# DhayaaAnbajagane/Baryonification

Measured on AMD Instinct MI355X. Metric: halos/sec for BaryonifyShell NSIDE=1024 (1000000-halo synthetic catalog), higher is better.
Workload: dtype f64 throughout in the parity-grade mode: f64 ring-row geometry, f64 pair math with 1e-11 elementary functions (fp32 seeds + one Newton step), f64 LDS accumulation, pix_offsets stored as two f32 arrays (hi + lo), f64 regrid geometry, f64 map

## Files before the change

baryonification_amd/csrc/bfgx_kernels.hpp:

```cpp
#pragma once
#include <hip/hip_runtime.h>
#include <stdint.h>
#include "bfgx_cosmo.hpp"
#include "bfgx_math.hpp"

namespace bfgx {

constexpr double kTwoPi    = 6.283185307179586476925286766559005768394;
constexpr double kHalfPi   = 1.570796326794896619231321691639751442099;
constexpr double kInvTwoPi = 1.0 / kTwoPi;
constexpr double kTwoThird = 2.0 / 3.0;
constexpr double kDeg2Rad  = kPi / 180.0;
constexpr double kRad2Deg  = 180.0 / kPi;

constexpr int kWave = 64;
constexpr int kWavesPerBlock = 4;
constexpr int kNC = 4;

enum { MODE_OFFSETS = 0, MODE_PAINT = 1, MODE_COUNT = 2 };

struct Hpx {
    int64_t nside, npix, ncap;
    double fact1, fact2;
};
// ... 87 lines not shown
        const int64_t iphi = 4 * iring + 1 - (ip - 2 * iring * (iring - 1));
        const double tmp = (double)(iring * iring) * h.fact2;
        z = tmp - 1.0;
        sth = (z < -0.99) ? sqrt(tmp * (2.0 - tmp)) : sqrt((1.0 - z) * (1.0 + z));
        phi = ((double)iphi - 0.5) * kHalfPi / (double)iring;
    }
}

template <bool WANT_W>
__device__ inline void get_interpol_ring(const Hpx &h, int64_t ir1, double theta, double phi, int64_t pix[4], double wgt[4])
{
    const int64_t ir2 = ir1 + 1;
    double theta1 = 0.0, theta2 = 0.0;
    pix[0] = pix[1] = pix[2] = pix[3] = 0;
    wgt[0] = wgt[1] = wgt[2] = wgt[3] = 0.0;
#pragma unroll
    for (int half = 0; half < 2; ++half) {
        const int64_t ir = half ? ir2 : ir1;
        if (half ? (ir < 4 * h.nside) : (ir > 0)) {
            int64_t sp, nr; bool shifted; double th = 0.0;
            if (WANT_W) ring_info2(h, ir, sp, nr, th, shifted);
            else ring_info_small(h, ir, sp, nr, shifted);
            const double dphi = kTwoPi / (double)nr;
            const double sh = shifted ? 0.5 : 0.0;
            const double tmp = phi / dphi - sh;
            int64_t i1 = (tmp < 0) ? (int64_t)tmp - 1 : (int64_t)tmp;
            const double w1 = (phi - ((double)i1 + sh) * dphi) / dphi;
            int64_t i2 = i1 + 1;
            if (i1 < 0) i1 += nr;
            if (i2 >= nr) i2 -= nr;
            pix[2 * half] = sp + i1; pix[2 * half + 1] = sp + i2;
            wgt[2 * half] = 1.0 - w1; wgt[2 * half + 1] = w1;
            if (half) theta2 = th; else theta1 = th;
        }
    }
    if (ir1 == 0) {
        const double wtheta = theta / theta2;
        wgt[2] *= wtheta; wgt[3] *= wtheta;
        const double fac = (1.0 - wtheta) * 0.25;
        wgt[0] = fac; wgt[1] = fac; wgt[2] += fac; wgt[3] += fac;
        pix[0] = (pix[2] + 2) & 3;
        pix[1] = (pix[3] + 2) & 3;
    } else if (ir2 == 4 * h.nside) {
        const double wtheta = (theta - theta1) / (kPi - theta1);
        wgt[0] *= (1.0 - wtheta); wgt[1] *= (1.0 - wtheta);
        const double fac = wtheta * 0.25;
        wgt[0] += fac; wgt[1] += fac; wgt[2] = fac; wgt[3] = fac;
        pix[2] = ((pix[0] + 2) & 3) + h.npix - 4;
        pix[3] = ((pix[1] + 2) & 3) + h.npix - 4;
    } else {
        const double wtheta = (theta - theta1) / (theta2 - theta1);
        wgt[0] *= (1.0 - wtheta); wgt[1] *= (1.0 - wtheta);
        wgt[2] *= wtheta; wgt[3] *= wtheta;
    }
}

template <bool WANT_W>
__device__ inline void get_interpol(const Hpx &h, double theta, double phi, int64_t pix[4], double wgt[4])
{
    get_interpol_ring<WANT_W>(h, ring_above(h, cos(theta)), theta, phi, pix, wgt);
}


struct RowSpan {
    int64_t start, nr;
    int32_t lo, cnt;
    bool shifted;
    double z, sth;
};

__device__ inline void disc_row_span(int nr, bool shifted, double z, double fnr, int ring, double z0, double xa, double cosr,
                                     double phi0, int irmin, int irmax, int &lo, int &cnt)
{
    lo = 0; cnt = 0;
    if (ring < irmin || ring > irmax) { cnt = nr; return; }
    const double x = (cosr - z * z0) * xa;
    const double ysq = 1.0 - z * z - x * x;
    if (!(ysq > 0.0)) return;
    const double dphi = atan2(sqrt(ysq), x);
    if (!(dphi > 0.0)) return;
    const double sh = shifted ? 0.5 : 0.0;
    const int64_t ip_lo = (int64_t)floor(fnr * (phi0 - dphi) - sh) + 1;
    const int64_t ip_hi = (int64_t)floor(fnr * (phi0 + dphi) - sh);
    int64_t c = ip_hi - ip_lo + 1;
    c = c < 0 ? 0 : (c > nr ? nr : c);
    cnt = (int)c;
    int64_t l = ip_lo;
    if (l < 0) l += nr;
    if (l >= nr) l -= nr;
    if (l < 0) l += nr;
    lo = (int)l;
}

__device__ inline void disc_row(const Hpx &h, int ring, double z0, double xa, double cosr, double phi0,
                                int irmin, int irmax, RowSpan &s)
{
    ring_info_small(h, ring, s.start, s.nr, s.shifted);
    ring_z_sth(h, ring, s.z, s.sth);
    s.lo = 0; s.cnt = 0;
    if (ring < irmin || ring > irmax) { s.cnt = (int)s.nr; return; }
    const double x = (cosr - s.z * z0) * xa;
    const double ysq = 1.0 - s.z * s.z - x * x;
    if (!(ysq > 0.0)) return;
    const double dphi = atan2(sqrt(ysq), x);
    if (!(dphi > 0.0)) return;
    const double sh = s.shifted ? 0.5 : 0.0;
    const double fnr = (double)s.nr * kInvTwoPi;
    const int64_t ip_lo = (int64_t)floor(fnr * (phi0 - dphi) - sh) + 1;
    const int64_t ip_hi = (int64_t)floor(fnr * (phi0 + dphi) - sh);
    int64_t c = ip_hi - ip_lo + 1;
    c = c < 0 ? 0 : (c > s.nr ? s.nr : c);
    s.cnt = (int)c;
    int64_t l = ip_lo;
    if (l < 0) l += s.nr;
    if (l >= s.nr) l -= s.nr;
    if (l < 0) l += s.nr;
    s.lo = (int)l;
}

__device__ inline void interp_neighbours(const Hpx &h, double theta, double phi, int32_t ring[4], int32_t k[4])
{
    int64_t pix[4]; double w[4];
    get_interpol<false>(h, theta, phi, pix, w);
    const double z = cos(theta);
    const int64_t ir1 = ring_above(h, z), ir2 = ir1 + 1;
    for (int q = 0; q < 4; ++q) {
        int64_t rg = (q < 2) ? ir1 : ir2;
        if (rg < 1) rg = 1;
        if (rg > 4 * h.nside - 1) rg = 4 * h.nside - 1;
        int64_t st, nr; bool sh;
        ring_info_small(h, rg, st, nr, sh);
        ring[q] = (int32_t)rg;
        k[q] = (int32_t)(pix[q] - st);
    }
}

struct DevTable {
    int32_t ndim;
    int32_t n[BFGX_MAX_DIM];
    const double *axis[BFGX_MAX_DIM];
    const double *values;
    const float *values32;
    int32_t rdelta, logv;
    double eps_model;
    int32_t r_uniform;
    double r0, inv_dr, r1;
};

struct PairTable {
    const double *values, *raxis;
    const float *values32;
    double r0, inv_dr, r1;
    int32_t nr, r_uniform, rdelta, _pad;
};

__host__ __device__ inline PairTable make_pair_table(const DevTable &t)
{
    PairTable p;
    p.values = t.values; p.raxis = t.axis[2]; p.values32 = t.values32;
    p.r0 = t.r0; p.inv_dr = t.inv_dr; p.r1 = t.r1;
    p.nr = t.n[2]; p.r_uniform = t.r_uniform; p.rdelta = t.rdelta; p._pad = 0;
    return p;
}

struct DevModel {
    DevTable tab;
    Background bg_runner, bg_model;
    bfgx_massdef md_runner, md_model;
    double eps_runner;
    int32_t same_model;
    const double *da_coef;
    double da_step;
};

constexpr int kNCmax = 16;
constexpr int kNCmaxShell = 4 << BFGX_MAX_EXTRA;
struct RowSetX {
    double w[kNCmaxShell];
    int32_t rowoff[kNCmaxShell];
};
struct ExtraCols { const double *p[BFGX_MAX_EXTRA]; };

struct alignas(16) HaloRec {
    double z0, xa, s0, phi0;
    double cph0, sph0;
    double cosr;
    double theta, phi;
    double D, a, inv_a, rcut, lnoff;
    double w[kNC];
    int32_t rowoff[kNC];
    int32_t irmin, irmax, rfirst, rlast;
    int32_t oob;
    int32_t allphi;
    int32_t fb;
    int32_t _pad;
    double flo, fhi;
    int32_t fb_ring[4], fb_k[4];
};

__device__ inline double dev_E2(const Background &b, double a)
{
    const double a3 = a * a * a;
    const double de = (b.w0 == -1.0) ? b.Omega_l : b.Omega_l * pow(a, -3.0 * (1.0 + b.w0));
    return b.Omega_m / a3 + de + b.Omega_r / (a3 * a);
}

__device__ inline double dev_radius(const Background &b, const bfgx_massdef &md, double M, double a)
{
    double rho = b.rho_crit0 * dev_E2(b, a);
    if (md.rho_type == 1) rho = b.rho_crit0 * b.Omega_m / (a * a * a);
    return cbrt(M / (4.18879020479 * md.Delta * rho));
}

__device__ inline int axis_find(const double *g, int n, double x)
{
    if (!(x >= g[0]) || !(x <= g[n - 1])) return -1;
    int lo = 0, hi = n - 1;
    while (hi - lo > 1) {
        const int mid = (lo + hi) >> 1;
        if (x >= g[mid]) lo = mid; else hi = mid;
    }
    return lo;
}

template <int NC>
__device__ inline bool table_corners(const DevTable &tab, const double *gz, const double *gm, double x0, double x1, const double *xe,
                                     double *wv, int32_t *ro)
{
    const int iz = axis_find(gz, tab.n[0], x0);
    const int im = axis_find(gm, tab.n[1], x1);
    constexpr int K = (NC == 4) ? 0 : (NC == 8 ? 1 : (NC == 16 ? 2 : (NC == 32 ? 3 : 4)));
    static_assert(NC == (4 << K), "NC = 4 * 2^K");
    int ip[K > 0 ? K : 1];
    double tp[K > 0 ? K : 1];
    bool oob = (iz < 0 || im < 0);
#pragma unroll
    for (int k = 0; k < K; ++k) {
        const double *g = tab.axis[3 + k];
        ip[k] = axis_find(g, tab.n[3 + k], xe[k]);
        tp[k] = 0.0;
        oob = oob || ip[k] < 0;
        if (ip[k] >= 0) tp[k] = (xe[k] - g[ip[k]]) / (g[ip[k] + 1] - g[ip[k]]);
    }
    if (!oob) {
        const double tz = (x0 - gz[iz]) / (gz[iz + 1] - gz[iz]);
        const double tm = (x1 - gm[im]) / (gm[im + 1] - gm[im]);
        const int nr = tab.n[2];
        for (int c = 0; c < NC; ++c) {
            const int bz = (c >> (K + 1)) & 1, bm = (c >> K) & 1;
            double w = (1.0 * (bz ? tz : 1.0 - tz)) * (bm ? tm : 1.0 - tm);
            int idx = (iz + bz) * tab.n[1] + im + bm;
#pragma unroll
            for (int k = 0; k < K; ++k) {
                const int b = (c >> (K - 1 - k)) & 1;
                w *= (b ? tp[k] : 1.0 - tp[k]);
                idx = idx * tab.n[3 + k] + ip[k] + b;
            }
            wv[c] = w;
            ro[c] = idx * nr;
        }
    } else {
        for (int c = 0; c < NC; ++c) { wv[c] = 0.0; ro[c] = 0; }
    }
    return oob;
}

struct Tiling {
    int32_t BR, W, nbands, ntiles;
    const int32_t *band_tile0;
    const int32_t *band_nphi;
    const int32_t *band_nrmin;
    const int32_t *tile_band;
    const int32_t *tile_order;
    const struct RingRec *rings;
};

__device__ inline int tile_ks(int j, int nr, int nphi) { return (int)(((unsigned)j * (unsigned)nr + (unsigned)nphi - 1u) / (unsigned)nphi); }

__device__ inline int ring_len(const Hpx &h, int ring)
{
    const int64_t n = h.nside;
    return (int)(4 * (ring < n ? ring : (ring > 3 * n ? 4 * n - ring : n)));
}

constexpr int kRefMax = 4;
struct TileRef {
    union {
        struct { int32_t tile[kRefMax], slot[kRefMax]; } few;
        struct { int32_t rfirst, rlast, allphi, _p; double flo, fhi; } many;
    };
    int32_t n;
    int32_t live;
    int32_t _pad[2];
};

enum { kClsNone = 0, kClsFast = 1, kClsGeneric = 2 };

struct DiscSpan {
    int32_t fb, rfirst, rlast, allphi;
    int32_t fb_ring[4], fb_k[4];
    double flo, fhi;
};

template <typename F>
__device__ inline void for_each_tile(const Hpx &h, const Tiling &T, const DiscSpan &r, F &&f)
{
    if (r.fb) {
        int seen[4], ns = 0;
        for (int q = 0; q < 4; ++q) {
            const int b = (r.fb_ring[q] - 1) / T.BR;
            const int nphi = T.band_nphi[b];
            const int t = T.band_tile0[b] + (int)(((int64_t)r.fb_k[q] * nphi) / ring_len(h, r.fb_ring[q]));
            bool dup = false;
            for (int i = 0; i < ns; ++i) dup |= (seen[i] == t);
            if (!dup) { seen[ns++] = t; f(t); }
        }
        return;
    }
    if (r.rlast < r.rfirst) return;
    const int b0 = (r.rfirst - 1) / T.BR, b1 = (r.rlast - 1) / T.BR;
    for (int b = b0; b <= b1; ++b) {
        const int nphi = T.band_nphi[b], t0 = T.band_tile0[b];
        bool all = r.allphi || nphi == 1;
        int jlo = 0, jhi = nphi - 1;
        if (!all) {
            const double margin = 2.0 * (double)nphi / (double)T.band_nrmin[b] + 1e-6;
            jlo = (int)floor((double)nphi * r.flo - margin);
            jhi = (int)floor((double)nphi * r.fhi + margin);
            if (jhi - jlo + 1 >= nphi) { all = true; jlo = 0; jhi = nphi - 1; }
        }
        for (int jj = jlo; jj <= jhi; ++jj) {
            int j = jj % nphi;
            if (j < 0) j += nphi;
            f(t0 + j);
        }
    }
}

struct alignas(16) RowRec {
    double z0, s0, xa, cosr, phi0;
    int32_t rfirst, rlast;
    int32_t fb;
    int32_t _pad;
    double cut2;
};
struct FbRec { int32_t ring[4], k[4]; };

template <typename real>
struct alignas(16) PairRecT {
    real scale2;
    real cut2;
    real aD;
    real cph0, sph0;
    real w[4];
    int32_t cell;
    int32_t oob;
    int32_t hidx, _pad;
};

template <typename real>
struct Tab8T {
    const real *v;
    real r0, r1, inv_dr;
    int32_t nr, _pad;
};

constexpr int kCntPadMax = 32;
struct RunSlot { int base, hr; };
__device__ inline RunSlot wave_run_issue(int32_t *cnt, int tile, bool active)
{
    RunSlot r;
    r.base = 0; r.hr = 0;
    if (__ballot(active) == 0ull) return r;
    const int lane = (int)__builtin_amdgcn_mbcnt_hi(~0u, __builtin_amdgcn_mbcnt_lo(~0u, 0u));
    const int key = active ? tile : -1 - lane;
    const int prev = __shfl_up(key, 1, kWave);
    const bool head = (lane == 0) || (key != prev);
    const unsigned long long hm = __ballot(head);
    const int hl = 63 - __clzll((long long)(hm & ((2ull << lane) - 1ull)));
    const unsigned long long up = (lane == kWave - 1) ? 0ull : (hm >> (lane + 1));
    const int next = up ? lane + __ffsll((long long)up) : kWave;
    r.hr = active ? (hl | ((lane - hl + 1) << 8)) : 0;
    if (head && active) r.base = atomicAdd(cnt + tile, next - lane);
    return r;
}
__device__ inline int wave_run_resolve(const RunSlot &r)
{
    const int b = __shfl(r.base, r.hr & 63, kWave);
    return r.hr ? b + (r.hr >> 8) - 1 : 0;
}

struct PrepOut {
    HaloRec *rec;
    RowSetX *rowsx;
    RowRec *rowrec;
    void *pairrec;
    FbRec *fbrec;
    TileRef *tref;
    int32_t *cnt_a, *cnt_b;
    int32_t *entries_a, *slow_list, *slow_cnt;
    float *work_est;
    int32_t cap_a;
    int32_t cnt_pad;
    int32_t fast;
    int32_t rec_all;
    int32_t ncell_m, nrm1;
    int64_t blk_rows, blk_stride;
};

template <int NC, typename real>
__device__ __forceinline__ void halo_prep_one(const DevModel &m, const Hpx &h, int64_t j, bool live, const double *gz, const double *gm,
                                              const double *__restrict__ M, const double *__restrict__ z,
                                              const double *__restrict__ ra, const double *__restrict__ dec,
                                              ExtraCols ex,
                                              const double *__restrict__ lnz1, const double *__restrict__ lnM,
                                              int fallback4, const Tiling &T, const PrepOut &o, int *s_nslow, float *s_work);

constexpr int kK0Occ = 4;
template <int NC, typename real>
__global__ void __launch_bounds__(256, kK0Occ)
halo_prep_kernel(DevModel m, Hpx h, int64_t nhalo,
                 const double *__restrict__ M, const double *__restrict__ z,
                 const double *__restrict__ ra, const double *__restrict__ dec,
                 ExtraCols ex,
                 const double *__restrict__ lnz1, const double *__restrict__ lnM,
                 int fallback4, Tiling T, PrepOut o)
{
    __shared__ int s_nslow;
    __shared__ float s_work;
    if (threadIdx.x == 0) { s_nslow = 0; s_work = 0.0f; }
    constexpr int kAxisLds = 128;
    __shared__ double ax_lds[2 * kAxisLds];
    const bool ax_in_lds = m.tab.n[0] <= kAxisLds && m.tab.n[1] <= kAxisLds;
    if (ax_in_lds) {
        for (int i = threadIdx.x; i < m.tab.n[0]; i += blockDim.x) ax_lds[i] = m.tab.axis[0][i];
        for (int i = threadIdx.x; i < m.tab.n[1]; i += blockDim.x) ax_lds[kAxisLds + i] = m.tab.axis[1][i];
        __syncthreads();
    }
    const double *gz = ax_in_lds ? ax_lds : m.tab.axis[0], *gm = ax_in_lds ? ax_lds + kAxisLds : m.tab.axis[1];
    constexpr int kBandLds = 1024;
    __shared__ int32_t band_lds[3 * kBandLds + 1];
    if (o.tref && T.nbands <= kBandLds) {
        for (int i = threadIdx.x; i <= T.nbands; i += blockDim.x) band_lds[i] = T.band_tile0[i];
        for (int i = threadIdx.x; i < T.nbands; i += blockDim.x) { band_lds[kBandLds + 1 + i] = T.band_nphi[i]; band_lds[2 * kBandLds + 1 + i] = T.band_nrmin[i]; }
        __syncthreads();
        T.band_tile0 = band_lds; T.band_nphi = band_lds + kBandLds + 1; T.band_nrmin = band_lds + 2 * kBandLds + 1;
    }
    __syncthreads();
    const int64_t j = (int64_t)blockIdx.x * blockDim.x + threadIdx.x;
    halo_prep_one<NC, real>(m, h, j < nhalo ? j : nhalo - 1, j < nhalo, gz, gm, M, z, ra, dec, ex, lnz1, lnM, fallback4, T, o, &s_nslow, &s_work);
    if (o.slow_cnt) {
        __syncthreads();
        if (threadIdx.x == 0) o.slow_cnt[blockIdx.x] = s_nslow;
        if (threadIdx.x == 0 && o.work_est) o.work_est[blockIdx.x] = s_work;
    }
}

template <int NC, typename real>
__device__ __forceinline__ void halo_prep_one(const DevModel &m, const Hpx &h, int64_t j, bool live, const double *gz, const double *gm,
                                              const double *__restrict__ M, const double *__restrict__ z,
                                              const double *__restrict__ ra, const double *__restrict__ dec,
                                              ExtraCols ex,
                                              const double *__restrict__ lnz1, const double *__restrict__ lnM,
                                              int fallback4, const Tiling &T, const PrepOut &o, int *s_nslow, float *s_work)
{
    HaloRec r;
    const int64_t jin = o.blk_rows > 0 ? (j / o.blk_rows) * o.blk_stride + (j % o.blk_rows) : j;
    const double M_j = M[jin], z_j = z[jin];
    const double a = 1.0 / (1.0 + z_j);
    const double R = dev_radius(m.bg_runner, m.md_runner, M_j, a);
    double D;
    {
        int i = (int)floor(z_j / m.da_step);
        i = max(0, min(i, kDaKnots - 2));
        const double t = z_j - (double)i * m.da_step;
        const double *c = m.da_coef + 4 * i;
        D = ((c[0] * t + c[1]) * t + c[2]) * t + c[3];
    }
    const double radius = R * m.eps_runner / D;

    const double theta = kHalfPi - dec[jin] * kDeg2Rad;
    const double phi = ra[jin] * kDeg2Rad;
    double st, ct, sp, cp;
    sincos_bounded(theta, st, ct);
    sincos_bounded(phi, sp, cp);
    const double thq = theta;
    double phq = phi - kTwoPi * floor(phi * kInvTwoPi);
    if (phq >= kTwoPi) phq -= kTwoPi;
    if (st == 0.0) phq = 0.0;
    r.z0 = ct;
    r.s0 = st;
    r.xa = 1.0 / sqrt((1.0 - r.z0) * (1.0 + r.z0));
    r.phi0 = phq;
    r.cph0 = cp; r.sph0 = sp;
    r.theta = theta; r.phi = phi;
    r.D = D; r.a = a;

    const int64_t nl4 = 4 * h.nside;
    bool pole = false;
    double sr_ = 0.0;
    const bool bad = !live || !(radius > 0.0) || !isfinite(radius) || !(theta >= 0.0) || !(theta <= kPi) || !isfinite(phi);
    if (bad) {
        r.cosr = 1.0; r.irmin = 1; r.irmax = 0; r.rfirst = 1; r.rlast = 0;
        r.z0 = 1.0; r.s0 = 0.0; r.xa = 1.0; r.phi0 = 0.0; r.cph0 = 1.0; r.sph0 = 0.0;
    } else if (radius >= kPi) {
        r.cosr = -1.0; r.irmin = (int32_t)nl4; r.irmax = 0; r.rfirst = 1; r.rlast = (int32_t)(nl4 - 1);
        pole = true;
    } else {
        double cr_;
        sincos_bounded(radius, sr_, cr_);
        r.cosr = cr_;
        const double rlat1 = thq - radius;
        const double rlat2 = thq + radius;
        int64_t irmin = ring_above(h, ct * cr_ + st * sr_) + 1;
        int64_t irmax = ring_above(h, ct * cr_ - st * sr_);
        if (irmax > nl4 - 1) irmax = nl4 - 1;
        r.irmin = (int32_t)irmin; r.irmax = (int32_t)irmax;
        r.rfirst = (int32_t)(((rlat1 <= 0) && (irmin > 1)) ? 1 : irmin);
        r.rlast = (int32_t)(((rlat2 >= kPi) && (irmax + 1 < nl4)) ? nl4 - 1 : irmax);
        pole = (rlat1 <= 0) || (rlat2 >= kPi);
    }
    double dmax;
    {
        const double sr = (radius >= kHalfPi) ? 1.0 : sr_;
        r.allphi = (pole || radius >= kHalfPi || !(sr < 0.999 * r.s0)) ? 1 : 0;
        const double xs = sr / r.s0, xs2 = xs * xs;
        const double as_small = xs * (1.0 + xs2 * (1.0 / 6.0 + xs2 * (3.0 / 40.0 + xs2 * (15.0 / 336.0 + xs2 * (105.0 / 3456.0)))));
        dmax = r.allphi ? kPi : (xs < 0.35 ? as_small * (1.0 + 2e-6) : asin(xs));
        r.flo = (phq - dmax) * kInvTwoPi;
        r.fhi = (phq + dmax) * kInvTwoPi;
    }

    r.fb = 0; r._pad = 0;
    for (int q = 0; q < 4; ++q) { r.fb_ring[q] = 0; r.fb_k[q] = 0; }
    if (fallback4 && !bad && (r.rlast - r.rfirst) < 8) {
        int total = 0;
        const int span = r.rlast - r.rfirst, mid = (r.rfirst + r.rlast) >> 1;
        for (int t = 0; t <= span && total < 4; ++t) {
            const int ring = mid + ((t & 1) ? ((t + 1) >> 1) : -(t >> 1));
            RowSpan s;
            disc_row(h, ring, r.z0, r.xa, r.cosr, r.phi0, r.irmin, r.irmax, s);
            total += s.cnt;
        }
        if (total < 4) {
            r.fb = 1;
            interp_neighbours(h, theta, phi, r.fb_ring, r.fb_k);
        }
    }

    const bool to_fast = o.fast && NC == 4;
    const int cls = bad ? kClsNone : (to_fast ? kClsFast : kClsGeneric);
    bool geo_wide = false;
    if (cls == kClsFast) {
        geo_wide = r.allphi || !(dmax <= 0.40);
        if (r.fb) for (int q = 0; q < 4; ++q) if (r.fb_ring[q] < 16 || r.fb_ring[q] > (int)nl4 - 16) geo_wide = true;
    }
    if (o.work_est) {
        float w = (cls == kClsFast) ? (r.fb ? 4.0f : (float)(radius * radius) * 0.25f * (float)h.npix) : 0.0f;
#pragma unroll
        for (int sft = kWave >> 1; sft > 0; sft >>= 1) w += __shfl_xor(w, sft, kWave);
        if ((threadIdx.x & (kWave - 1)) == 0) atomicAdd(s_work, w);
    }
    TileRef ref;
    RunSlot run[kRefMax];
    for (int i = 0; i < kRefMax; ++i) { run[i].base = 0; run[i].hr = 0; }
    ref.n = 0; ref.live = cls != kClsNone; ref._pad[0] = ref._pad[1] = 0;
    for (int i = 0; i < kRefMax; ++i) { ref.few.tile[i] = 0; ref.few.slot[i] = 0; }
    if (o.tref) {
        DiscSpan ds;
        ds.fb = r.fb; ds.rfirst = r.rfirst; ds.rlast = r.rlast; ds.allphi = r.allphi; ds.flo = r.flo; ds.fhi = r.fhi;
        for (int q = 0; q < 4; ++q) { ds.fb_ring[q] = r.fb_ring[q]; ds.fb_k[q] = r.fb_k[q]; }
        int tl[kRefMax] = {0, 0, 0, 0};
        int nt = 0;
        if (cls != kClsNone) for_each_tile(h, T, ds, [&](int t) { if (nt < kRefMax) tl[nt] = t; ++nt; });
        ref.n = nt;
#pragma unroll
        for (int i = 0; i < kRefMax; ++i) {
            run[i] = wave_run_issue(o.cnt_a, tl[i] * o.cnt_pad, nt <= kRefMax && i < nt && cls == kClsFast);
            if (nt <= kRefMax) { ref.few.tile[i] = (i < nt) ? tl[i] : 0; ref.few.slot[i] = 0; }
        }
        if (nt <= kRefMax) {
            for (int i = 0; i < kRefMax; ++i)
                if (i < nt && cls == kClsGeneric) { ref.few.slot[i] = -1; atomicAdd(o.cnt_b + tl[i], 1); }
        } else {
            ref.many.rfirst = r.rfirst; ref.many.rlast = r.rlast; ref.many.allphi = r.allphi; ref.many._p = 0;
            ref.many.flo = r.flo; ref.many.fhi = r.fhi;
            for_each_tile(h, T, ds, [&](int t) { atomicAdd(o.cnt_b + t, 1); });
        }
    }
    const double Rmod = (m.same_model ? R : dev_radius(m.bg_model, m.md_model, M_j, a)) / a;
    r.rcut = m.tab.eps_model * Rmod;
    r.inv_a = 1.0 / a;
    const double x0 = lnz1 ? lnz1[jin] : fast_log(1.0 / a), x1 = lnM ? lnM[jin] : fast_log(M_j);
    r.lnoff = m.tab.rdelta ? (x0 - fast_log(Rmod)) : x0;
    double wv[NC];
    int32_t ro[NC];
    double xe[BFGX_MAX_EXTRA];
#pragma unroll
    for (int k = 0; k < BFGX_MAX_EXTRA; ++k) xe[k] = ((4 << k) < NC) ? ex.p[k][jin] : 0.0;
    const bool oob = table_corners<NC>(m.tab, gz, gm, x0, x1, xe, wv, ro);
    r.oob = oob ? 1 : 0;
    if (NC == 4) {
        for (int c = 0; c < 4; ++c) { r.w[c] = wv[c]; r.rowoff[c] = ro[c]; }
    } else {
        for (int c = 0; c < 4; ++c) { r.w[c] = 0.0; r.rowoff[c] = 0; }
        RowSetX rx;
        for (int c = 0; c < kNCmaxShell; ++c) { rx.w[c] = c < NC ? wv[c] : 0.0; rx.rowoff[c] = c < NC ? ro[c] : 0; }
        if (live) o.rowsx[j] = rx;
    }

    if (live && o.rec && (o.rec_all || cls == kClsGeneric)) o.rec[j] = r;
    if (cls == kClsFast) {
        RowRec rr;
        rr.z0 = r.z0; rr.s0 = r.s0; rr.xa = r.xa; rr.cosr = r.cosr; rr.phi0 = r.phi0;
        rr.rfirst = r.rfirst; rr.rlast = r.rlast; rr.fb = (r.fb ? 1 : 0) | (geo_wide ? 2 : 0); rr._pad = 0;
        const double cut = r.rcut * a / D;
        rr.cut2 = cut * cut;
        double sh, chh;
        sincos_bounded(0.5 * fmin(radius, kPi), sh, chh);
        const bool implied = (m.tab.logv != 0) || (!r.fb && cut >= 2.0 * sh * (1.0 + 1e-9));
        o.rowrec[j] = rr;
        PairRecT<real> pr;
        double scl = D * r.inv_a;
        if (m.tab.rdelta) scl /= Rmod;
        pr.scale2 = oob ? (real)1.0e30 : (real)(scl * scl);
        pr.cut2 = implied ? (real)0 : (real)(1.0 / rr.cut2);
        pr.aD = (real)(a / D);
        pr.cph0 = (real)r.cph0; pr.sph0 = (real)r.sph0;
        for (int c = 0; c < 4; ++c) pr.w[c] = (real)wv[c < NC ? c : 0];
        const int nr = o.nrm1 + 1, nm = o.ncell_m + 1;
        const int row0 = oob ? 0 : ro[0] / nr;
        const int iz = row0 / nm, im = row0 - iz * nm;
        pr.cell = (iz * o.ncell_m + im) * o.nrm1 * 8;
        pr.oob = oob ? 1 : 0;
        pr.hidx = (int32_t)j; pr._pad = 0;
        reinterpret_cast<PairRecT<real> *>(o.pairrec)[j] = pr;
        if (r.fb || geo_wide) {
            FbRec f;
            for (int q = 0; q < 4; ++q) { f.ring[q] = r.fb_ring[q]; f.k[q] = r.fb_k[q]; }
            if (!r.fb) { f.ring[0] = r.irmin; f.ring[1] = r.irmax; }
            o.fbrec[j] = f;
        }
    }
    if (o.tref) {
#pragma unroll
        for (int i = 0; i < kRefMax; ++i) {
            const int sl = wave_run_resolve(run[i]);
            if (ref.n <= kRefMax && cls == kClsFast && i < ref.n) ref.few.slot[i] = sl;
        }
        bool slow = (cls != kClsNone) && (ref.n > kRefMax || cls != kClsFast);
        if (cls == kClsFast && ref.n <= kRefMax) {
            for (int i = 0; i < kRefMax; ++i) if (i < ref.n) {
                const int sl = ref.few.slot[i];
                if (sl < o.cap_a) o.entries_a[(int64_t)ref.few.tile[i] * o.cap_a + sl] = (int32_t)j;
                else { ref.few.slot[i] = -1; atomicAdd(o.cnt_b + ref.few.tile[i], 1); slow = true; }
            }
        }
        if (live && slow) o.tref[j] = ref;
        if (slow) o.slow_list[(int64_t)blockIdx.x * 256 + atomicAdd(s_nslow, 1)] = (int32_t)j;
    }
}

__global__ void __launch_bounds__(256)
disc_rings_kernel(DevModel m, Hpx h, int64_t nhalo, const double *__restrict__ M, const double *__restrict__ z,
                  const double *__restrict__ dec, int32_t *__restrict__ rings, int margin)
{
    const int64_t j = (int64_t)blockIdx.x * blockDim.x + threadIdx.x;
    if (j >= nhalo) return;
    const double M_j = M[j], z_j = z[j];
    const double a = 1.0 / (1.0 + z_j);
    const double R = dev_radius(m.bg_runner, m.md_runner, M_j, a);
    double D;
    {
        int i = (int)floor(z_j / m.da_step);
        i = max(0, min(i, kDaKnots - 2));
        const double t = z_j - (double)i * m.da_step;
        const double *c = m.da_coef + 4 * i;
        D = ((c[0] * t + c[1]) * t + c[2]) * t + c[3];
    }
    const double radius = R * m.eps_runner / D;
    const double theta = kHalfPi - dec[j] * kDeg2Rad;
    const int nl4 = (int)(4 * h.nside);
    int first = 1, last = 0;
    const bool bad = !(radius > 0.0) || !isfinite(radius) || !(theta >= 0.0) || !(theta <= kPi) || !(M_j > 0.0) || !isfinite(M_j) || !(z_j > -1.0);
    if (!bad) {
        if (radius >= kPi) { first = 1; last = nl4 - 1; }
        else {
            const double lo = fmax(theta - radius, 0.0), hi = fmin(theta + radius, kPi);
            first = (int)ring_above(h, cos(lo)) - 1;
            last = (int)ring_above(h, cos(hi)) + 2;
            first = max(1, first - 1); last = min(nl4 - 1, last + 1);
        }
        first = max(1, first - margin); last = min(nl4 - 1, last + margin);
    }
    rings[2 * j] = first; rings[2 * j + 1] = last;
}

constexpr int kRouteMaxRanks = 64, kRouteMaxCols = 8;
struct RouteArgs {
    int32_t world, ncols;
    int32_t bounds[kRouteMaxRanks + 1];
    int64_t start[kRouteMaxRanks];
    const double *col[kRouteMaxCols];
    int64_t blockcap;
    int32_t *overflow;
};

__device__ inline void route_range(const RouteArgs &a, int first, int last, int &jlo, int &jhi)
{
    jlo = 0; jhi = -1;
    if (first > last) return;
    while (jlo < a.world - 1 && a.bounds[jlo + 1] <= first) ++jlo;
    jhi = jlo;
    while (jhi < a.world - 1 && a.bounds[jhi + 1] <= last) ++jhi;
}

constexpr int kRouteGrid = 512;
template <bool FILL>
__global__ void __launch_bounds__(256)
route_halos_kernel(RouteArgs a, int64_t n, const int32_t *__restrict__ rings, int32_t *__restrict__ counts, int32_t *__restrict__ cursor,
                   double *__restrict__ rows)
{
    __shared__ int hist[kRouteMaxRanks], base[kRouteMaxRanks], taken[kRouteMaxRanks];
    const int tid = threadIdx.x;
    if (tid < kRouteMaxRanks) { hist[tid] = 0; taken[tid] = 0; }
    __syncthreads();
    const int64_t per = (n + gridDim.x - 1) / gridDim.x;
    const int64_t j0 = (int64_t)blockIdx.x * per, j1 = min(n, j0 + per);
    for (int64_t j = j0 + tid; j < j1; j += 256) {
        int jlo, jhi;
        route_range(a, rings[2 * j], rings[2 * j + 1], jlo, jhi);
        for (int d = jlo; d <= jhi; ++d) atomicAdd(&hist[d], 1);
    }
    __syncthreads();
    if (!FILL) {
        if (tid < a.world && hist[tid]) atomicAdd(counts + tid, hist[tid]);
        return;
    }
    if (tid < a.world) base[tid] = hist[tid] ? atomicAdd(cursor + tid, hist[tid]) : 0;
    __syncthreads();
    for (int64_t j = j0 + tid; j < j1; j += 256) {
        int jlo, jhi;
        route_range(a, rings[2 * j], rings[2 * j + 1], jlo, jhi);
        for (int d = jlo; d <= jhi; ++d) {
            const int64_t slot = base[d] + atomicAdd(&taken[d], 1);
            if (a.blockcap > 0) {
                if (slot >= a.blockcap) { *a.overflow = 1; continue; }
                double *blk = rows + (int64_t)d * a.ncols * a.blockcap + slot;
                for (int c = 0; c < a.ncols; ++c) blk[c * a.blockcap] = a.col[c][j];
            } else {
                double *row = rows + (a.start[d] + slot) * a.ncols;
                for (int c = 0; c < a.ncols; ++c) row[c] = a.col[c][j];
            }
        }
    }
}

__global__ void __launch_bounds__(256)
route_blank_kernel(int32_t world, int32_t ncols, int64_t blockcap, double *__restrict__ rows)
{
    const int64_t n = (int64_t)world * blockcap;
    for (int64_t i = (int64_t)blockIdx.x * 256 + threadIdx.x; i < n; i += (int64_t)gridDim.x * 256)
        rows[(i / blockcap) * ncols * blockcap + (i % blockcap)] = __builtin_nan("");
}

struct RouteStepArgs {
    RouteArgs r;
    int32_t rank, margin;
    const double *M, *z, *dec;
    double *send, *recv;
};
__global__ void __launch_bounds__(256)
route_prepare_kernel(int32_t world, int32_t ncols, int64_t blockcap, double *__restrict__ send, double *__restrict__ recv, int32_t *__restrict__ cursor)
{
    if (blockIdx.x == 0 && (int)threadIdx.x < world) cursor[threadIdx.x] = 0;
    const int64_t nb = (int64_t)(world - 1) * blockcap, nr = (int64_t)world * blockcap;
    for (int64_t i = (int64_t)blockIdx.x * 256 + threadIdx.x; i < nb + nr; i += (int64_t)gridDim.x * 256) {
        double *base = i < nb ? send : recv;
        const int64_t k = i < nb ? i : i - nb;
        base[(k / blockcap) * ncols * blockcap + (k % blockcap)] = __builtin_nan("");
    }
}
__global__ void __launch_bounds__(256)
route_step_kernel(RouteStepArgs s, DevModel m, Hpx h, int64_t n, int32_t *__restrict__ cursor)
{
    const RouteArgs &a = s.r;
    __shared__ int hist[kRouteMaxRanks], base[kRouteMaxRanks], taken[kRouteMaxRanks];
    const int tid = threadIdx.x;
    if (tid < kRouteMaxRanks) { hist[tid] = 0; taken[tid] = 0; }
    __syncthreads();
    const int64_t per = (n + gridDim.x - 1) / gridDim.x;
    const int64_t j0 = (int64_t)blockIdx.x * per, j1 = min(n, j0 + per);
    const int nl4 = (int)(4 * h.nside);
    auto ring_range = [&](int64_t j, int &first, int &last) {
        const double M_j = s.M[j], z_j = s.z[j];
        const double aa = 1.0 / (1.0 + z_j);
        const double R = dev_radius(m.bg_runner, m.md_runner, M_j, aa);
        double D;
        {
            int i = (int)floor(z_j / m.da_step);
            i = max(0, min(i, kDaKnots - 2));
            const double t = z_j - (double)i * m.da_step;
            const double *c = m.da_coef + 4 * i;
            D = ((c[0] * t + c[1]) * t + c[2]) * t + c[3];
        }
        const double radius = R * m.eps_runner / D;
        const double theta = kHalfPi - s.dec[j] * kDeg2Rad;
        first = 1; last = 0;
        const bool bad = !(radius > 0.0) || !isfinite(radius) || !(theta >= 0.0) || !(theta <= kPi) || !(M_j > 0.0) || !isfinite(M_j) || !(z_j > -1.0);
        if (bad) return;
        if (radius >= kPi) { first = 1; last = nl4 - 1; }
        else {
            const double lo = fmax(theta - radius, 0.0), hi = fmin(theta + radius, kPi);
            first = (int)ring_above(h, cos(lo)) - 1;
            last = (int)ring_above(h, cos(hi)) + 2;
            first = max(1, first - 1); last = min(nl4 - 1, last + 1);
        }
        first = max(1, first - s.margin); last = min(nl4 - 1, last + s.margin);
    };
    constexpr int kStash = 4096;
    __shared__ int2 stash[kStash];
    for (int64_t j = j0 + tid; j < j1; j += 256) {
        int first, last, jlo, jhi;
        ring_range(j, first, last);
        if (j - j0 < kStash) stash[j - j0] = make_int2(first, last);
        route_range(a, first, last, jlo, jhi);
        for (int d = jlo; d <= jhi; ++d) atomicAdd(&hist[d], 1);
    }
    __syncthreads();
    if (tid < a.world) base[tid] = hist[tid] ? atomicAdd(cursor + tid, hist[tid]) : 0;
    __syncthreads();
    for (int64_t j = j0 + tid; j < j1; j += 256) {
        int first, last, jlo, jhi;
        if (j - j0 < kStash) { const int2 q = stash[j - j0]; first = q.x; last = q.y; } else ring_range(j, first, last);
        route_range(a, first, last, jlo, jhi);
        for (int d = jlo; d <= jhi; ++d) {
            const int64_t slot = base[d] + atomicAdd(&taken[d], 1);
            if (slot >= a.blockcap) { *a.overflow = 1; continue; }
            double *blk = (d == s.rank) ? s.recv + (int64_t)(a.world - 1) * a.ncols * a.blockcap
                                        : s.send + (int64_t)(d < s.rank ? d : d - 1) * a.ncols * a.blockcap;
            blk += slot;
            for (int c = 0; c < a.ncols; ++c) blk[c * a.blockcap] = a.col[c][j];
        }
    }
}

__global__ void __launch_bounds__(1024)
k1_form_kernel(int nblk, const float *__restrict__ work_est, float thr_total, int32_t *__restrict__ form)
{
    __shared__ float red[1024 / kWave];
    float s = 0.0f;
    for (int i = threadIdx.x; i < nblk; i += 1024) s += work_est[i];
#pragma unroll
    for (int sft = kWave >> 1; sft > 0; sft >>= 1) s += __shfl_xor(s, sft, kWave);
    if ((threadIdx.x & (kWave - 1)) == 0) red[threadIdx.x / kWave] = s;
    __syncthreads();
    if (threadIdx.x == 0) {
        float t = 0.0f;
        for (int w = 0; w < 1024 / kWave; ++w) t += red[w];
        form[0] = t >= thr_total ? 1 : 0;
    }
}

__global__ void __launch_bounds__(1024)
tile_scan_kernel(int ntiles, const int32_t *__restrict__ cnt, int32_t *__restrict__ start)
{
    constexpr int kPer = 8;
    __shared__ int32_t wtot[1024 / kWave];
    __shared__ int32_t carry;
    const int tid = threadIdx.x, lane = tid & (kWave - 1), wid = tid / kWave;
    if (tid == 0) carry = 0;
    __syncthreads();
    for (int base = 0; base < ntiles; base += 1024 * kPer) {
        const int lo = min(base + tid * kPer, ntiles), hi = min(lo + kPer, ntiles);
        int32_t c[kPer], s = 0;
#pragma unroll
        for (int q = 0; q < kPer; ++q) {
            const int i = lo + q;
            c[q] = i < hi ? cnt[i] : 0;
            s += c[q];
        }
        int32_t is = s;
#pragma unroll
        for (int off = 1; off < kWave; off <<= 1) {
            const int32_t us = __shfl_up(is, off, kWave);
            if (lane >= off) is += us;
        }
        if (lane == kWave - 1) wtot[wid] = is;
        __syncthreads();
        int32_t ps = carry;
        for (int w = 0; w < wid; ++w) ps += wtot[w];
        int32_t run = ps + is - s;
#pragma unroll
        for (int q = 0; q < kPer; ++q) {
            const int i = lo + q;
            if (i < hi) { start[i] = run; run += c[q]; }
        }
        __syncthreads();
        if (tid == 1023) carry = run;
        __syncthreads();
    }
    if (tid == 0) start[ntiles] = carry;
}

constexpr int kScanTilesPerWg = 1024 * 8;
template <int PHASE>
__global__ void __launch_bounds__(1024)
tile_scan_part_kernel(int ntiles, const int32_t *__restrict__ cnt, int32_t *__restrict__ start,
                      int32_t *__restrict__ block_tot, const int32_t *__restrict__ block_off)
{
    constexpr int kPer = 8;
    __shared__ int32_t wtot[1024 / kWave];
    const int tid = threadIdx.x, lane = tid & (kWave - 1), wid = tid / kWave;
    const int base = blockIdx.x * kScanTilesPerWg;
    const int lo = min(base + tid * kPer, ntiles), hi = min(lo + kPer, ntiles);
    int32_t c[kPer], s = 0;
#pragma unroll
    for (int q = 0; q < kPer; ++q) {
        const int i = lo + q;
        c[q] = i < hi ? cnt[i] : 0;
        s += c[q];
    }
    int32_t is = s;
#pragma unroll
    for (int off = 1; off < kWave; off <<= 1) {
        const int32_t us = __shfl_up(is, off, kWave);
        if (lane >= off) is += us;
    }
    if (lane == kWave - 1) wtot[wid] = is;
    __syncthreads();
    int32_t ps = 0;
    for (int w = 0; w < wid; ++w) ps += wtot[w];
    if (PHASE == 0) {
        if (tid == 1023) block_tot[blockIdx.x] = ps + is;
        return;
    }
    int32_t run = block_off[blockIdx.x] + ps + is - s;
#pragma unroll
    for (int q = 0; q < kPer; ++q) {
        const int i = lo + q;
        if (i < hi) { start[i] = run; run += c[q]; }
    }
}

__global__ void __launch_bounds__(1024)
tile_scan_blocks_kernel(int nblocks, int ntiles, const int32_t *__restrict__ block_tot, int32_t *__restrict__ block_off,
                        int32_t *__restrict__ start)
{
    __shared__ int32_t sa[1024];
    const int tid = threadIdx.x;
    sa[tid] = tid < nblocks ? block_tot[tid] : 0;
    __syncthreads();
    if (tid == 0) {
        int32_t ra = 0;
        for (int b = 0; b < nblocks; ++b) { block_off[b] = ra; ra += sa[b]; }
        start[ntiles] = ra;
    }
}

__global__ void __launch_bounds__(256)
tile_place_kernel(Hpx h, Tiling T, int64_t nhalo, const TileRef *__restrict__ tref,
                  const int32_t *__restrict__ start, int32_t *__restrict__ cur_b,
                  int32_t *__restrict__ entries, int64_t capacity, int32_t *__restrict__ overflow,
                  const int32_t *__restrict__ slow_list, const int32_t *__restrict__ slow_cnt)
{
    if ((int)threadIdx.x >= slow_cnt[blockIdx.x]) return;
    const int64_t j = slow_list[(int64_t)blockIdx.x * blockDim.x + threadIdx.x];
    if (j >= nhalo) return;
    const TileRef ref = tref[j];
    if (!ref.live) return;
    auto put = [&](int t) {
        const int64_t pos = (int64_t)start[t] + atomicAdd(cur_b + t, 1);
        if (pos < capacity) entries[pos] = (int32_t)j; else *overflow = 1;
    };
    if (ref.n <= kRefMax) {
        for (int i = 0; i < kRefMax; ++i)
            if (i < ref.n && ref.few.slot[i] < 0) put(ref.few.tile[i]);
    } else {
        DiscSpan ds;
        ds.fb = 0; ds.rfirst = ref.many.rfirst; ds.rlast = ref.many.rlast; ds.allphi = ref.many.allphi;
        ds.flo = ref.many.flo; ds.fhi = ref.many.fhi;
        for (int q = 0; q < 4; ++q) { ds.fb_ring[q] = 0; ds.fb_k[q] = 0; }
        for_each_tile(h, T, ds, put);
    }
}

template <typename ACC> __device__ inline void atomic_accumulate(ACC *p, double v) { atomicAdd(p, (ACC)v); }

template <int NC>
__device__ inline double radial_readout(const PairTable &t, const int32_t *rowoff, const double *w, double lx)
{
    const int n = t.nr;
    if (!(lx >= t.r0) || !(lx <= t.r1)) return __builtin_nan("");
    int i;
    double tr;
    if (t.r_uniform) {
        const double u = (lx - t.r0) * t.inv_dr;
        i = min((int)u, n - 2);
        tr = u - (double)i;
    } else {
        const double *g = t.raxis;
        int lo = 0, hi = n - 1;
        while (hi - lo > 1) { const int mid = (lo + hi) >> 1; if (lx >= g[mid]) lo = mid; else hi = mid; }
        i = lo;
        tr = (lx - g[i]) / (g[i + 1] - g[i]);
    }
    const double t0 = 1.0 - tr;
    double val = 0.0;
#pragma unroll
    for (int c = 0; c < NC; ++c) {
        const double *row = t.values + rowoff[c] + i;
        val = val + row[0] * (w[c] * t0);
        val = val + row[1] * (w[c] * tr);
    }
    return val;
}

template <int NC>
struct PairHaloT {
    double z0, s0, phi0, cph0, sph0, D, a, inv_a, rcut;
    double lnoff;
    double w[NC];
    int32_t rowoff[NC];
    int32_t oob, hidx;
};
using PairHalo = PairHaloT<kNC>;

template <int NC>
__device__ inline void load_pair_halo(PairHaloT<NC> &p, const HaloRec &r, int hidx, const RowSetX *rowsx = nullptr)
{
    p.z0 = r.z0; p.s0 = r.s0; p.phi0 = r.phi0; p.cph0 = r.cph0; p.sph0 = r.sph0;
    p.D = r.D; p.a = r.a; p.inv_a = r.inv_a; p.rcut = r.rcut; p.lnoff = r.lnoff;
    if (NC == kNC) {
        for (int c = 0; c < kNC; ++c) { p.w[c] = r.w[c]; p.rowoff[c] = r.rowoff[c]; }
    } else {
        const RowSetX &x = rowsx[hidx];
        for (int c = 0; c < NC; ++c) { p.w[c] = x.w[c]; p.rowoff[c] = x.rowoff[c]; }
    }
    p.oob = r.oob; p.hidx = hidx;
}

template <int MODE, int NC>
__device__ inline bool pair_value(const PairTable &tab, const PairHaloT<NC> &r, double z, double sth, double phi_pix, double v[3])
{
    double sd, cd;
    sincos_dphi(phi_pix - r.phi0, sd, cd);
    const double vx = sth * cd, vy = sth * sd, vz = z;
    const double dx = r.D * (vx - r.s0), dy = r.D * vy, dz = r.D * (vz - r.z0);
    const double r2 = dx * dx + dy * dy + dz * dz;
    if (!(r2 > 0.0)) return false;
    const double inv_r = fast_rsq(r2);
    const double r_sep = r2 * inv_r;
    const double r_com = r_sep * r.inv_a;
    const double lx = __builtin_fma(0.5, fast_log(r2), r.lnoff);
    double d = r.oob ? __builtin_nan("") : radial_readout<NC>(tab, r.rowoff, r.w, lx);
    if (MODE == MODE_PAINT) {
        const double paint = fast_exp(d);
        v[0] = paint;
        return isfinite(paint) && paint != 0.0;
    }
    if (!(r_com < r.rcut)) d = 0.0;
    if (!isfinite(d) || d == 0.0) return false;
    d *= r.a * inv_r;
    const double ox = d * dx, oy = d * dy, oz = d * dz;
    const double nx = __builtin_fma(r.D, vx, ox), ny = __builtin_fma(r.D, vy, oy), nz = __builtin_fma(r.D, vz, oz);
    const double inv_n = fast_rsq(nx * nx + ny * ny + nz * nz);
    const double ex = __builtin_fma(nx, inv_n, -vx), ey = __builtin_fma(ny, inv_n, -vy);
    v[2] = __builtin_fma(nz, inv_n, -vz);
    v[0] = ex * r.cph0 - ey * r.sph0;
    v[1] = ex * r.sph0 + ey * r.cph0;
    return true;
}

template <int MODE, int NC>
__device__ inline bool pair_value_fast(const PairTable &tab, const PairHaloT<NC> &r, double z, double sth, double x, double v[3])
{
    double sd, cd;
    sincos_small(x, sd, cd);
    const double vx = sth * cd, vy = sth * sd, vz = z;
    const double dx = r.D * (vx - r.s0), dy = r.D * vy, dz = r.D * (vz - r.z0);
    const double r2 = dx * dx + dy * dy + dz * dz;
    bool ok = (r2 > 0.0) && !r.oob;
    const double r2s = (r2 > 0.0) ? r2 : 1.0;
    const double inv_r = fast_rsq(r2s);
    const double r_com = r2s * inv_r * r.inv_a;
    const double lx = __builtin_fma(0.5, fast_log(r2s), r.lnoff);
    ok = ok && (lx >= tab.r0) && (lx <= tab.r1);
    const double u = (lx - tab.r0) * tab.inv_dr;
    const int i = max(0, min((int)u, tab.nr - 2));
    const double tr = u - (double)i, t0 = 1.0 - tr;
    double d = 0.0;
#pragma unroll
    for (int c = 0; c < NC; ++c) {
        const double *row = tab.values + r.rowoff[c] + i;
        d = d + row[0] * (r.w[c] * t0);
        d = d + row[1] * (r.w[c] * tr);
    }
    if (MODE == MODE_PAINT) {
        const double paint = fast_exp(d);
        v[0] = paint;
        return ok && isfinite(paint) && paint != 0.0;
    }
    ok = ok && (r_com < r.rcut) && isfinite(d) && d != 0.0;
    d *= r.a * inv_r;
    const double ox = d * dx, oy = d * dy, oz = d * dz;
    const double nx = __builtin_fma(r.D, vx, ox), ny = __builtin_fma(r.D, vy, oy), nz = __builtin_fma(r.D, vz, oz);
    const double inv_n = fast_rsq(nx * nx + ny * ny + nz * nz);
    const double ex = __builtin_fma(nx, inv_n, -vx), ey = __builtin_fma(ny, inv_n, -vy);
    v[2] = __builtin_fma(nz, inv_n, -vz);
    v[0] = ex * r.cph0 - ey * r.sph0;
    v[1] = ex * r.sph0 + ey * r.cph0;
    return ok;
}

__device__ inline double fold_dphi(double x)
{
    x = (x > kPi) ? x - kTwoPi : x;
    return (x < -kPi) ? x + kTwoPi : x;
}

struct RowLds {
    int32_t prefix[kWave];
    int32_t nr[kWave];
    int32_t lo[kWave];
    int64_t start[kWave];
    double z[kWave], sth[kWave], shift[kWave];
};

__device__ inline int wave_scan_incl(int v, int lane)
{
#pragma unroll
    for (int s = 1; s < kWave; s <<= 1) {
        const int u = __shfl_up(v, s, kWave);
        if (lane >= s) v += u;
    }
    return v;
}

__device__ inline uint32_t wave_scan_incl_u32(uint32_t v, int lane)
{
#pragma unroll
    for (int s = 1; s < kWave; s <<= 1) {
        const uint32_t u = __shfl_up(v, s, kWave);
        if (lane >= s) v += u;
    }
    return v;
}

template <int NC>
__device__ inline bool pair_value_fast32(const PairTable &tab, const PairHaloT<NC> &r, double z, double sth, double x, double v[3])
{
    double sd, cd;
    sincos_small(x, sd, cd);
    const double vx = sth * cd, vy = sth * sd;
    const double dx = r.D * (vx - r.s0), dy = r.D * vy, dz = r.D * (z - r.z0);
    const double r2 = dx * dx + dy * dy + dz * dz;
    const double rc = r.rcut * r.a;
    bool ok = (r2 > 0.0) && !r.oob && (r2 < rc * rc);
    const float r2f = (float)((r2 > 0.0) ? r2 : 1.0);
    float inv_r = __builtin_amdgcn_rsqf(r2f);
    inv_r = inv_r * __builtin_fmaf(-0.5f * r2f * inv_r, inv_r, 1.5f);
    const float lx = __builtin_fmaf(0.34657359027997264f, __builtin_amdgcn_logf(r2f), (float)r.lnoff);
    const float r0f = (float)tab.r0;
    ok = ok && (lx >= r0f) && (lx <= (float)tab.r1);
    const float u = (lx - r0f) * (float)tab.inv_dr;
    const int i = max(0, min((int)u, tab.nr - 2));
    const float tr = u - (float)i, t0 = 1.0f - tr;
    float d = 0.0f;
#pragma unroll
    for (int c = 0; c < NC; ++c) {
        const float *row = tab.values32 + r.rowoff[c] + i;
        const float w = (float)r.w[c];
        d = __builtin_fmaf(row[0], w * t0, d);
        d = __builtin_fmaf(row[1], w * tr, d);
    }
    ok = ok && isfinite(d) && d != 0.0f;
    const float sc = d * (float)r.a * inv_r * __builtin_amdgcn_rcpf((float)r.D);
    const float ex0 = sc * (float)dx, ey0 = sc * (float)dy, ez0 = sc * (float)dz;
    const float fx = (float)vx, fy = (float)vy, fz = (float)z;
    const float t = 2.0f * (fx * ex0 + fy * ey0 + fz * ez0) + (ex0 * ex0 + ey0 * ey0 + ez0 * ez0);
    const float g = t * __builtin_fmaf(t, __builtin_fmaf(t, -0.3125f, 0.375f), -0.5f);
    const float ex = __builtin_fmaf(g, fx + ex0, ex0), ey = __builtin_fmaf(g, fy + ey0, ey0), ez = __builtin_fmaf(g, fz + ez0, ez0);
    const float cp = (float)r.cph0, sp = (float)r.sph0;
    v[0] = (double)(ex * cp - ey * sp);
    v[1] = (double)(ex * sp + ey * cp);
    v[2] = (double)ez;
    return ok;
}

template <int MODE, typename ACC>
__global__ void __launch_bounds__(kWave * kWavesPerBlock)
halo_scatter_kernel(PairTable pt, Hpx h, int64_t nhalo, const HaloRec *__restrict__ recs,
                    ACC *__restrict__ out, int64_t *__restrict__ counts)
{
    __shared__ RowLds lds[kWavesPerBlock];
    const int lane = threadIdx.x & (kWave - 1);
    const int wid = __builtin_amdgcn_readfirstlane(threadIdx.x / kWave);
    const int64_t j = (int64_t)blockIdx.x * kWavesPerBlock + wid;
    if (j >= nhalo) return;
    RowLds &L = lds[wid];
    const HaloRec &r = recs[j];
    PairHalo ph;
    load_pair_halo(ph, r, (int)j);
    constexpr int NCOMP = (MODE == MODE_OFFSETS) ? 3 : 1;

    int64_t npairs = 0;
    if (r.fb) {
        npairs = 4;
        if (MODE != MODE_COUNT && lane < 4) {
            int64_t st, nr; bool sh; double z, sth, v[3];
            ring_info_small(h, r.fb_ring[lane], st, nr, sh);
            ring_z_sth(h, r.fb_ring[lane], z, sth);
            const double phi_pix = ((double)r.fb_k[lane] + (sh ? 0.5 : 0.0)) * (kTwoPi / (double)nr);
            if (pair_value<MODE, kNC>(pt, ph, z, sth, phi_pix, v)) {
                ACC *o = out + NCOMP * (st + r.fb_k[lane]);
                for (int c = 0; c < NCOMP; ++c) atomic_accumulate(o + c, v[c]);
            }
        }
    } else {
        for (int rbase = r.rfirst; rbase <= r.rlast; rbase += kWave) {
            const int ring = rbase + lane;
            RowSpan s;
            s.cnt = 0; s.lo = 0; s.start = 0; s.nr = 1; s.shifted = false; s.z = 0.0; s.sth = 0.0;
            if (ring <= r.rlast) disc_row(h, ring, r.z0, r.xa, r.cosr, r.phi0, r.irmin, r.irmax, s);
            const int incl = wave_scan_incl(s.cnt, lane);
            const int total = __shfl(incl, kWave - 1, kWave);
            L.prefix[lane] = incl - s.cnt;
            L.nr[lane] = (int)s.nr; L.lo[lane] = s.lo; L.start[lane] = s.start;
            L.z[lane] = s.z; L.sth[lane] = s.sth; L.shift[lane] = s.shifted ? 0.5 : 0.0;
            __builtin_amdgcn_wave_barrier();
            npairs += total;
            if (MODE != MODE_COUNT) {
                for (int t = lane; t < total; t += kWave) {
                    int row = 0;
#pragma unroll
                    for (int st = kWave >> 1; st > 0; st >>= 1)
                        if (L.prefix[row + st] <= t) row += st;
                    const int nrr = L.nr[row];
                    int k = L.lo[row] + (t - L.prefix[row]);
                    if (k >= nrr) k -= nrr;
                    const double phi_pix = ((double)k + L.shift[row]) * (kTwoPi / (double)nrr);
                    double v[3];
                    if (pair_value<MODE, kNC>(pt, ph, L.z[row], L.sth[row], phi_pix, v)) {
                        ACC *o = out + NCOMP * (L.start[row] + k);
                        for (int c = 0; c < NCOMP; ++c) atomic_accumulate(o + c, v[c]);
                    }
                }
            }
            __builtin_amdgcn_wave_barrier();
        }
    }
    if (counts && lane == 0) counts[j] = npairs;
}

template <int WHAT>
__global__ void __launch_bounds__(kWave * kWavesPerBlock)
halo_pairs_kernel(Hpx h, int64_t nhalo, const HaloRec *__restrict__ recs, const int64_t *__restrict__ off, const double *__restrict__ vals,
                  double *__restrict__ r_out, double *__restrict__ out)
{
    __shared__ RowLds lds[kWavesPerBlock];
    const int lane = threadIdx.x & (kWave - 1);
    const int wid = __builtin_amdgcn_readfirstlane(threadIdx.x / kWave);
    const int64_t j = (int64_t)blockIdx.x * kWavesPerBlock + wid;
    if (j >= nhalo) return;
    RowLds &L = lds[wid];
    const HaloRec &r = recs[j];
    const int64_t base = off[j];
    auto pair = [&](int64_t q, int64_t pix, double z, double sth, double phi_pix) {
        double sd, cd;
        sincos_dphi(phi_pix - r.phi0, sd, cd);
        const double vx = sth * cd, vy = sth * sd, vz = z;
        const double dx = r.D * (vx - r.s0), dy = r.D * vy, dz = r.D * (vz - r.z0);
        const double r_sep = sqrt(dx * dx + dy * dy + dz * dz);
        if (WHAT == 0) { r_out[q] = r_sep * r.inv_a; return; }
        const double val = vals[q];
        if (WHAT == 2) {
            if (isfinite(val) && val != 0.0) atomic_accumulate(out + pix, val);
            return;
        }
        const double d = val * r.a;
        double ox = d * (dx / r_sep), oy = d * (dy / r_sep), oz = d * (dz / r_sep);
        ox = isfinite(ox) ? ox : 0.0; oy = isfinite(oy) ? oy : 0.0; oz = isfinite(oz) ? oz : 0.0;
        if (ox == 0.0 && oy == 0.0 && oz == 0.0) return;
        const double nx = __builtin_fma(r.D, vx, ox), ny = __builtin_fma(r.D, vy, oy), nz = __builtin_fma(r.D, vz, oz);
        const double inv_n = 1.0 / sqrt(nx * nx + ny * ny + nz * nz);
        const double ex = __builtin_fma(nx, inv_n, -vx), ey = __builtin_fma(ny, inv_n, -vy), ez = __builtin_fma(nz, inv_n, -vz);
// ... 460 lines not shown
```

Baseline: 924.7 million.

## Spread large-disc tile placement across wave lanes; unroll per-lane tile lists

In tile_place_kernel, halos that cover many tiles are now processed one at a time by the whole wave. Each lane computes a band span, a wave prefix scan sums the tile counts, and lanes binary-search for their tile. This replaces serial per-thread loops that caused heavy divergence. Separately, the dynamic-index writes into the small seen/tl arrays become unrolled select-writes so they can stay in registers instead of scratch memory. The cost is extra shuffle work and serialization over the large halos in each wave.

```diff
diff --git a/baryonification_amd/csrc/bfgx_kernels.hpp b/baryonification_amd/csrc/bfgx_kernels.hpp
--- a/baryonification_amd/csrc/bfgx_kernels.hpp
+++ b/baryonification_amd/csrc/bfgx_kernels.hpp
@@ -413,38 +413,56 @@
     double flo, fhi;
 };
 
+struct BandSpan { int32_t t0, nphi, jlo, cnt; };
+__device__ inline BandSpan band_span(const Tiling &T, const DiscSpan &r, int b)
+{
+    BandSpan s;
+    s.nphi = T.band_nphi[b]; s.t0 = T.band_tile0[b];
+    bool all = r.allphi || s.nphi == 1;
+    int jlo = 0, jhi = s.nphi - 1;
+    if (!all) {
+        const double margin = 2.0 * (double)s.nphi / (double)T.band_nrmin[b] + 1e-6;
+        jlo = (int)floor((double)s.nphi * r.flo - margin);
+        jhi = (int)floor((double)s.nphi * r.fhi + margin);
+        if (jhi - jlo + 1 >= s.nphi) { all = true; jlo = 0; jhi = s.nphi - 1; }
+    }
+    s.jlo = jlo; s.cnt = jhi - jlo + 1;
+    return s;
+}
+__device__ inline int band_span_tile(const BandSpan &s, int k)
+{
+    int j = (s.jlo + k) % s.nphi;
+    if (j < 0) j += s.nphi;
+    return s.t0 + j;
+}
+
 template <typename F>
 __device__ inline void for_each_tile(const Hpx &h, const Tiling &T, const DiscSpan &r, F &&f)
 {
     if (r.fb) {
-        int seen[4], ns = 0;
+        int seen[4] = {0, 0, 0, 0}, ns = 0;
+#pragma unroll
         for (int q = 0; q < 4; ++q) {
             const int b = (r.fb_ring[q] - 1) / T.BR;
             const int nphi = T.band_nphi[b];
             const int t = T.band_tile0[b] + (int)(((int64_t)r.fb_k[q] * nphi) / ring_len(h, r.fb_ring[q]));
             bool dup = false;
-            for (int i = 0; i < ns; ++i) dup |= (seen[i] == t);
-            if (!dup) { seen[ns++] = t; f(t); }
+#pragma unroll
+            for (int i = 0; i < 4; ++i) dup |= (i < ns) && (seen[i] == t);
+            if (!dup) {
+#pragma unroll
+                for (int i = 0; i < 4; ++i) seen[i] = (i == ns) ? t : seen[i];
+                ++ns;
+                f(t);
+            }
         }
         return;
     }
     if (r.rlast < r.rfirst) return;
     const int b0 = (r.rfirst - 1) / T.BR, b1 = (r.rlast - 1) / T.BR;
     for (int b = b0; b <= b1; ++b) {
-        const int nphi = T.band_nphi[b], t0 = T.band_tile0[b];
-        bool all = r.allphi || nphi == 1;
-        int jlo = 0, jhi = nphi - 1;
-        if (!all) {
-            const double margin = 2.0 * (double)nphi / (double)T.band_nrmin[b] + 1e-6;
-            jlo = (int)floor((double)nphi * r.flo - margin);
-            jhi = (int)floor((double)nphi * r.fhi + margin);
-            if (jhi - jlo + 1 >= nphi) { all = true; jlo = 0; jhi = nphi - 1; }
-        }
-        for (int jj = jlo; jj <= jhi; ++jj) {
-            int j = jj % nphi;
-            if (j < 0) j += nphi;
-            f(t0 + j);
-        }
+        const BandSpan s = band_span(T, r, b);
+        for (int k = 0; k < s.cnt; ++k) f(band_span_tile(s, k));
     }
 }
 
@@ -683,7 +701,11 @@
         for (int q = 0; q < 4; ++q) { ds.fb_ring[q] = r.fb_ring[q]; ds.fb_k[q] = r.fb_k[q]; }
         int tl[kRefMax] = {0, 0, 0, 0};
         int nt = 0;
-        if (cls != kClsNone) for_each_tile(h, T, ds, [&](int t) { if (nt < kRefMax) tl[nt] = t; ++nt; });
+        if (cls != kClsNone) for_each_tile(h, T, ds, [&](int t) {
+#pragma unroll
+            for (int i = 0; i < kRefMax; ++i) tl[i] = (i == nt) ? t : tl[i];
+            ++nt;
+        });
         ref.n = nt;
 #pragma unroll
         for (int i = 0; i < kRefMax; ++i) {
@@ -1075,24 +1097,62 @@
                   int32_t *__restrict__ entries, int64_t capacity, int32_t *__restrict__ overflow,
                   const int32_t *__restrict__ slow_list, const int32_t *__restrict__ slow_cnt)
 {
-    if ((int)threadIdx.x >= slow_cnt[blockIdx.x]) return;
-    const int64_t j = slow_list[(int64_t)blockIdx.x * blockDim.x + threadIdx.x];
-    if (j >= nhalo) return;
-    const TileRef ref = tref[j];
-    if (!ref.live) return;
-    auto put = [&](int t) {
+    const int nslow = slow_cnt[blockIdx.x];
+    if (nslow == 0) return;
+    const int lane = (int)__builtin_amdgcn_mbcnt_hi(~0u, __builtin_amdgcn_mbcnt_lo(~0u, 0u));
+    const bool mine = (int)threadIdx.x < nslow;
+    const int64_t j = mine ? (int64_t)slow_list[(int64_t)blockIdx.x * blockDim.x + threadIdx.x] : nhalo;
+    TileRef ref;
+    ref.n = 0; ref.live = 0;
+    for (int i = 0; i < kRefMax; ++i) { ref.few.tile[i] = 0; ref.few.slot[i] = 0; }
+    if (j < nhalo) ref = tref[j];
+    const bool act = j < nhalo && ref.live != 0;
+    auto put = [&](int t, int32_t halo) {
         const int64_t pos = (int64_t)start[t] + atomicAdd(cur_b + t, 1);
-        if (pos < capacity) entries[pos] = (int32_t)j; else *overflow = 1;
+        if (pos < capacity) entries[pos] = halo; else *overflow = 1;
     };
-    if (ref.n <= kRefMax) {
+    if (act && ref.n <= kRefMax) {
         for (int i = 0; i < kRefMax; ++i)
-            if (i < ref.n && ref.few.slot[i] < 0) put(ref.few.tile[i]);
-    } else {
+            if (i < ref.n && ref.few.slot[i] < 0) put(ref.few.tile[i], (int32_t)j);
+    }
+    unsigned long long many = __ballot(act && ref.n > kRefMax);
+    while (many) {
+        const int src = __ffsll((long long)many) - 1;
+        many &= many - 1ull;
         DiscSpan ds;
-        ds.fb = 0; ds.rfirst = ref.many.rfirst; ds.rlast = ref.many.rlast; ds.allphi = ref.many.allphi;
-        ds.flo = ref.many.flo; ds.fhi = ref.many.fhi;
+        ds.fb = 0; ds.rfirst = __shfl(ref.many.rfirst, src, kWave); ds.rlast = __shfl(ref.many.rlast, src, kWave);
+        ds.allphi = __shfl(ref.many.allphi, src, kWave);
+        ds.flo = __shfl(ref.many.flo, src, kWave); ds.fhi = __shfl(ref.many.fhi, src, kWave);
         for (int q = 0; q < 4; ++q) { ds.fb_ring[q] = 0; ds.fb_k[q] = 0; }
-        for_each_tile(h, T, ds, put);
+        const int32_t halo = __shfl((int32_t)j, src, kWave);
+        if (ds.rlast < ds.rfirst) continue;
+        const int b0 = (ds.rfirst - 1) / T.BR, b1 = (ds.rlast - 1) / T.BR;
+        for (int bb = b0; bb <= b1; bb += kWave) {
+            BandSpan s;
+            s.t0 = 0; s.nphi = 1; s.jlo = 0; s.cnt = 0;
+            if (bb + lane <= b1) s = band_span(T, ds, bb + lane);
+            if (s.cnt < 0) s.cnt = 0;
+            int incl = s.cnt;
+#pragma unroll
+            for (int off = 1; off < kWave; off <<= 1) {
+                const int up = __shfl_up(incl, off, kWave);
+                if (lane >= off) incl += up;
+            }
+            const int total = __shfl(incl, kWave - 1, kWave), excl = incl - s.cnt;
+            for (int base = 0; base < total; base += kWave) {
+                const int i = base + lane;
+                int kb = 0;
+#pragma unroll
+                for (int step = kWave >> 1; step > 0; step >>= 1) {
+                    const int e = __shfl(excl, kb + step, kWave);
+                    if (e <= i) kb += step;
+                }
+                BandSpan sb;
+                sb.t0 = __shfl(s.t0, kb, kWave); sb.nphi = __shfl(s.nphi, kb, kWave); sb.jlo = __shfl(s.jlo, kb, kWave); sb.cnt = 0;
+                const int k = i - __shfl(excl, kb, kWave);
+                if (i < total) put(band_span_tile(sb, k), halo);
+            }
+        }
     }
 }
 
```

Result: faster. 937.2 million (median of 6 runs) (+1.3%).
